# PKU-EPIC/PartManip

Measured on AMD Instinct MI355X. Metric: PPO env-steps/sec (whole node), 4096 envs x 1024-pt clouds, higher is better.
Workload: dtype f32

## Files before the change

### partmanip_amd/csrc/pointnet_enc_screen.h

```cpp
#pragma once

typedef _Float16 ps_f16x8 __attribute__((ext_vector_type(8)));

#define PS_LDP (PN_C2 + 8)
#define PS_CAP 256
#define PS_NW 8
#define PS_P3 (16 * 16 * 64 * 8)
#define PS_OFF_P3 0
#define PS_OFF_W3 (2 * PS_P3)
#define PS_OFF_EPS (PS_OFF_W3 + PN_C3 * PN_C2 * 4)
#define PS_OFF_INV (PS_OFF_EPS + PN_C3 * 4)
#define PS_PACKED_BYTES (PS_OFF_INV + PN_C3 * 4)
#ifndef PS_ABLATE
#define PS_ABLATE 0
#endif
#ifndef PS_SCHED_DEFAULT
#define PS_SCHED_DEFAULT 0
#endif

extern "C" size_t pm_pointnet_packed_screen_bytes(void) { return PS_PACKED_BYTES; }

__device__ __forceinline__ unsigned ps_cvt_pk(float a, float b) {
    unsigned r;
    asm("v_cvt_pk_f16_f32 %0, %1, %2" : "=v"(r) : "v"(a), "v"(b));
    return r;
}

__global__ __launch_bounds__(PN_C2) void ps_pack_kernel(const float* __restrict__ W3, const float* __restrict__ b3,
                                                         unsigned char* __restrict__ packed) {
    __shared__ double Ls[PN_C2], Rs[PN_C2], Ss[PN_C2];
    __shared__ float Ms[PN_C2];
    const int c = blockIdx.x, k = threadIdx.x;
    const float w = W3[c * PN_C2 + k];
    const float aw = fabsf(w);
    Ls[k] = (double)aw;
    Ms[k] = aw < INFINITY ? aw : 0.f;
    __syncthreads();
    for (int o = PN_C2 / 2; o > 0; o >>= 1) {
        if (k < o) {
            Ls[k] += Ls[k + o];
            Ms[k] = fmaxf(Ms[k], Ms[k + o]);
        }
        __syncthreads();
    }
    int ex = -200;
    if (Ms[0] > 0.f) frexpf(Ms[0], &ex);
    const int s = min(15 - ex, 126);
    const float ws = ldexpf(w, s);
    const _Float16 w16 = (_Float16)ws;
    const float wf = (float)w16, d = fabsf(ws - wf);
    Rs[k] = (double)(fabsf(wf) < 0x1p-14f ? fmaxf(fabsf(ws), d) : d);
    Ss[k] = (double)fabsf(wf);
    __syncthreads();
    for (int o = PN_C2 / 2; o > 0; o >>= 1) {
        if (k < o) {
            Rs[k] += Rs[k + o];
            Ss[k] += Ss[k + o];
        }
        __syncthreads();
    }
    const int nb = c >> 5, li = c & 31, step = k >> 4, lq = (k >> 3) & 1, e = k & 7;
    ((_Float16*)(packed + PS_OFF_P3))[(((nb * 16 + step) * 64) + lq * 32 + li) * 8 + e] = w16;
    ((float*)(packed + PS_OFF_W3))[c * PN_C2 + k] = w;
    if (k == 0) {
        const double ed = ((Rs[0] + 0x1p-12 * Ss[0]) * ldexp(1.0, -s) + 1024.0 * 0x1p-24 * (Ls[0] + fabs((double)b3[c]))) * (1.0 + 0x1p-10) + 0x1p-116;
        float ef = (float)ed;
        if ((double)ef < ed) ef = __uint_as_float(__float_as_uint(ef) + 1);
        ((float*)(packed + PS_OFF_EPS))[c] = ef;
        ((float*)(packed + PS_OFF_INV))[c] = ldexpf(1.f, -s);
    }
}

extern "C" int pm_pointnet_pack_weights_screen(const float* W3, const float* b3, void* packed, void* stream) {
    PM_REQUIRE(W3 && b3 && packed);
    if (((uintptr_t)packed & 15) != 0) return PM_EALIGN;
    hipLaunchKernelGGL(ps_pack_kernel, dim3(PN_C3), dim3(PN_C2), 0, pm_stream(stream), W3, b3, (unsigned char*)packed);
    PM_CHECK_LAUNCH();
    return PM_OK;
}

#define PS_MFMA(a, b, c) __builtin_amdgcn_mfma_f32_32x32x16_f16((a), (b), (c), 0, 0, 0)
__device__ __forceinline__ ps_f16x8 ps_h(const uint4& v) { return *(const ps_f16x8*)&v; }

__device__ __forceinline__ void ps_stream(const unsigned short* __restrict__ A, const uint4* __restrict__ B, f32x16 (&acc)[2][2]) {
    uint4 b0[2], b1[2], b2[2], b3[2], a0[2], a1[2];
#pragma unroll
    for (int nb = 0; nb < 2; ++nb) {
        b0[nb] = B[(size_t)(nb * 16 + 0) * 64];
        b1[nb] = B[(size_t)(nb * 16 + 1) * 64];
        b2[nb] = B[(size_t)(nb * 16 + 2) * 64];
    }
#pragma unroll
    for (int mb = 0; mb < 2; ++mb) a0[mb] = *(const uint4*)(A + mb * 32 * PS_LDP);
#define PS_STEP(S_, AC, AN, BC, BN, PFA, PFB)                                                  \
    {                                                                                          \
        if (PFA) {                                                                             \
            _Pragma("unroll") for (int mb = 0; mb < 2; ++mb)                                   \
                AN[mb] = *(const uint4*)(A + mb * 32 * PS_LDP + ((S_) + 1) * 16);              \
        }                                                                                      \
        if (PFB) {                                                                             \
            _Pragma("unroll") for (int nb = 0; nb < 2; ++nb)                                   \
                BN[nb] = B[(size_t)(nb * 16 + (S_) + 3) * 64];                                 \
        }                                                                                      \
        __builtin_amdgcn_sched_barrier(0);                                                     \
        _Pragma("unroll") for (int nb = 0; nb < 2; ++nb)                                       \
            _Pragma("unroll") for (int mb = 0; mb < 2; ++mb)                                   \
                acc[mb][nb] = PS_MFMA(ps_h(AC[mb]), ps_h(BC[nb]), acc[mb][nb]);                \
        __builtin_amdgcn_sched_barrier(0);                                                     \
    }
#pragma unroll 1
    for (int s = 0; s < 12; s += 4) {
        PS_STEP(s, a0, a1, b0, b3, 1, 1)
        PS_STEP(s + 1, a1, a0, b1, b0, 1, 1)
        PS_STEP(s + 2, a0, a1, b2, b1, 1, 1)
        PS_STEP(s + 3, a1, a0, b3, b2, 1, 1)
    }
    PS_STEP(12, a0, a1, b0, b3, 1, 1)
    PS_STEP(13, a1, a0, b1, b0, 1, 0)
    PS_STEP(14, a0, a1, b2, b1, 1, 0)
    PS_STEP(15, a1, a0, b3, b2, 0, 0)
#undef PS_STEP
}

template <int SCHED>
__device__ __forceinline__ bool ps_late_wave(int wave) { return SCHED == 1 && __builtin_amdgcn_readfirstlane(wave) >= 4; }

template <int NT>
__device__ __forceinline__ void ps_copy_h2(const float* __restrict__ H, float* __restrict__ dst, int tid) {
#pragma unroll 2
    for (int i = 0; i < PN_TM * PN_C2 / 4 / NT; ++i) {
        const int q = tid + NT * i, row = q >> 6, c4 = q & 63;
        const f32x4 v = *(const f32x4*)(H + row * PN_LD2 + 4 * c4);
        *(f32x4*)(dst + row * PN_C2 + 4 * c4) = v;
    }
}

static_assert(PN_TM * PN_MAXC == PS_NW * 64, "one staged slot per thread");
__device__ __forceinline__ float ps_point_load(const float* __restrict__ xb, int tile, int C, int tid) {
    const int p = tid >> 3, d = tid & 7;
    return d < C ? xb[(tile * PN_TM + p) * C + d] : 0.f;
}
__device__ __forceinline__ void ps_point_store(float v, int sub_mean, const float (&cen)[3], int tid, float* __restrict__ Xs) {
    const int d = tid & 7;
    if (sub_mean && d < 3) v -= cen[d];
    Xs[tid] = v;
}

#ifdef PS_PROFILE
__device__ unsigned long long ps_prof[4 * 16 * PS_NW * 16];
extern "C" int pm_debug_ps_prof_read(void* dst) {
    return hipMemcpyFromSymbol(dst, HIP_SYMBOL(ps_prof), sizeof(ps_prof)) == hipSuccess ? 0 : 1;
}
#define PS_STAMP(i)                                                                                         \
    if (b < 4 && tile < 16 && lane0 == 0) ps_prof[((b * 16 + tile) * PS_NW + wave) * 16 + (i)] = __builtin_readcyclecounter()
#else
#define PS_STAMP(i)
#endif

template <int CT, int SCHED>
__global__ __launch_bounds__(PS_NW * 64, 2) void pn_fwd_screen_kernel(
    const float* __restrict__ x, long ldx, int P, int C, int sub_mean, const float* __restrict__ W1,
    const float* __restrict__ b1, const float* __restrict__ b2, const float* __restrict__ b3,
    const float* __restrict__ packed, const unsigned char* __restrict__ packed_s, int max_mean, float* __restrict__ feat,
    long ldf, int32_t* __restrict__ argmax, float* __restrict__ h2_save, unsigned long long* __restrict__ counters) {
    constexpr int NT = PS_NW * 64;
    __shared__ __attribute__((aligned(16))) float H[PN_TM * PN_LD2];
    __shared__ __attribute__((aligned(16))) unsigned short Hh[PN_TM * PS_LDP];
    __shared__ __attribute__((aligned(16))) float Xs[PN_TM * PN_MAXC];
    __shared__ double red[16];
    __shared__ double cs[PN_C2];
    __shared__ int skey[PS_NW][PS_CAP];

    const int b = blockIdx.x, tid = threadIdx.x, lane0 = tid & 63, wave = tid >> 6;
    const float* xb = x + (long)b * ldx;
    const float4* P2v = (const float4*)(packed + PN_P2_OFF);
    const float4* P3v = (const float4*)(packed + PN_P3_OFF);
    const uint4* S3 = (const uint4*)(packed_s + PS_OFF_P3);
    const float* W3r = (const float*)(packed_s + PS_OFF_W3);
    const float* epsg = (const float*)(packed_s + PS_OFF_EPS);
    const float* invg = (const float*)(packed_s + PS_OFF_INV);

    float cen[3] = {0.f, 0.f, 0.f};
    if (sub_mean) cloud_centroid<NT>(xb, P, C, red, cen);

    float vmax = -INFINITY, pois = 0.f;
    int imax = 0;
    double csum = 0.0;

    const int li0 = lane0 & 31;
    const float b2r = b2[wave * 32 + li0];
    const float b3r[2] = {b3[(wave * 2 + 0) * 32 + li0], b3[(wave * 2 + 1) * 32 + li0]};
    const float epsr[2] = {epsg[(wave * 2 + 0) * 32 + li0], epsg[(wave * 2 + 1) * 32 + li0]};
    const float invr[2] = {invg[(wave * 2 + 0) * 32 + li0], invg[(wave * 2 + 1) * 32 + li0]};
    float w1r[4] = {0.f, 0.f, 0.f, 0.f}, b1r = 0.f;
    if constexpr (CT == 3 || CT == 4) layer1_row<CT>(W1, b1, w1r, b1r);

    const int ntiles = P / PN_TM;
    stage_points<PN_TM, NT>(xb, 0, C, sub_mean, cen, Xs);
    for (int tile = 0; tile < ntiles; ++tile) {
        int lane = lane0;
        asm volatile("" : "+v"(lane));
        const int li = lane & 31, lh = lane >> 5;
        PS_STAMP(0);
        __syncthreads();
        float xnext = 0.f;
        if (tile + 1 < ntiles) xnext = ps_point_load(xb, tile + 1, C, tid);
        if (!(PS_ABLATE & 1)) {
            if constexpr (CT == 3 || CT == 4) layer1_tile<CT, PN_TM, NT, true>(Xs, w1r, b1r, H);
            else layer1_tile<CT, PN_TM, NT, true>(Xs, W1, b1, C, H);
        }
        PS_STAMP(1);
        __syncthreads();
        {
            f32x16 acc2[2][1];
            zero_acc<2, 1>(acc2);
            if (PS_ABLATE & 2) {
#pragma unroll
                for (int mb = 0; mb < 2; ++mb)
#pragma unroll
                    for (int r = 0; r < 16; ++r)
                        acc2[mb][0][r] = H[(mb * 32 + (r & 3) + 8 * (r >> 2) + 4 * lh) * PN_LD1 + ((wave * 32 + li) & 127)];
            } else {
                layer2_mfma<2, 1>(H, P2v, wave, lane, acc2);
            }
            PS_STAMP(2);
            __syncthreads();
            PS_STAMP(3);
            const int col = wave * 32 + li;
            const float b2c = b2r;
            float ts = 0.f;
            const bool planes = !(PS_ABLATE & 8) || tile == 0;
            const bool odd = (lane & 1) != 0;
            unsigned* Hh2 = (unsigned*)(Hh + (odd ? PS_LDP : 0) + (col & ~1));
#pragma unroll
            for (int mb = 0; mb < 2; ++mb)
#pragma unroll
                for (int r = 0; r < 16; r += 2) {
                    const float z0 = acc2[mb][0][r] + b2c, z1 = acc2[mb][0][r + 1] + b2c;
                    f32x2 v2;
                    if (PS_ABLATE & 4) {
                        v2.x = z0;
                        v2.y = z1;
                    } else {
                        v2 = pm_tanh2(z0, z1);
                    }
                    const int row0 = mb * 32 + (r & 3) + 8 * (r >> 2) + 4 * lh;
                    H[row0 * PN_LD2 + col] = v2.x;
                    H[(row0 + 1) * PN_LD2 + col] = v2.y;
                    ts += v2.x;
                    ts += v2.y;
                    const float own = odd ? v2.y : v2.x, send = odd ? v2.x : v2.y;
                    const float recv = __int_as_float(__builtin_amdgcn_update_dpp(0, __float_as_int(send), 0xB1, 0xf, 0xf, false));
                    const float a = odd ? recv : own, c = odd ? own : recv;
                    if (planes) Hh2[row0 * (PS_LDP / 2)] = ps_cvt_pk(a, c);
                }
            ts += __shfl_xor(ts, 32, 64);
            csum += (double)ts;
            if (tile + 1 < ntiles) ps_point_store(xnext, sub_mean, cen, tid, Xs);
        }
        PS_STAMP(4);
        __syncthreads();
        PS_STAMP(5);

        const bool copy = h2_save && !(PS_ABLATE & 128), late = ps_late_wave<SCHED>(wave);
        float* h2dst = copy ? h2_save + ((long)b * P + (long)tile * PN_TM) * PN_C2 : nullptr;
        if (copy && late) ps_copy_h2<NT>(H, h2dst, tid);

        f32x16 acc[2][2];
        if (PS_ABLATE & 16) {
#pragma unroll
            for (int nb = 0; nb < 2; ++nb)
#pragma unroll
                for (int mb = 0; mb < 2; ++mb)
#pragma unroll
                    for (int r = 0; r < 16; ++r)
                        acc[mb][nb][r] = b3r[nb] + H[(mb * 32 + (r & 3) + 8 * (r >> 2) + 4 * lh) * PN_LD2 + ((wave * 64 + nb * 32 + li) & 255)];
        } else {
            zero_acc<2, 2>(acc);
            ps_stream(Hh + li * PS_LDP + lh * 8, S3 + (size_t)(wave * 2 * 16) * 64 + lane, acc);
        }
        PS_STAMP(6);

        unsigned msk[2];
        float tmax[2];
#if (PS_ABLATE & 32) && defined(__HIP_DEVICE_COMPILE__)
#pragma unroll
        for (int nb = 0; nb < 2; ++nb) {
#pragma unroll
            for (int mb = 0; mb < 2; ++mb) asm volatile("" ::"v"(acc[mb][nb]));
            msk[nb] = 0;
            tmax[nb] = 0.f;
        }
#else
#pragma unroll
        for (int nb = 0; nb < 2; ++nb) {
            float m = -INFINITY;
            const float iv = invr[nb], b3c = b3r[nb];
#pragma unroll
            for (int mb = 0; mb < 2; ++mb)
#pragma unroll
                for (int r = 0; r < 16; ++r) {
                    if (!(PS_ABLATE & 16)) acc[mb][nb][r] = fmaf(acc[mb][nb][r], iv, b3c);
                    m = fmaxf(m, acc[mb][nb][r]);
                }
            m = fmaxf(m, __shfl_xor(m, 32, 64));
            const float e = epsr[nb];
            const float vm = __shfl(vmax, nb * 32 + li, 64);
            const float thr = m - 2.f * e;
            unsigned k = 0;
#pragma unroll
            for (int mb = 0; mb < 2; ++mb)
#pragma unroll
                for (int r = 0; r < 16; ++r) {
                    const float z = acc[mb][nb][r];
                    const bool s = !(z < thr) && !(z + e <= vm);
                    k |= (s ? 1u : 0u) << (mb * 16 + r);
                }
            msk[nb] = k;
            tmax[nb] = m;
        }
#endif
        const int n = __popc(msk[0]) + __popc(msk[1]);
        int incl = n;
#pragma unroll
        for (int o = 1; o < 64; o <<= 1) {
            const int t = __shfl_up(incl, o, 64);
            if (lane >= o) incl += t;
        }
        const int total = __builtin_amdgcn_readlane(incl, 63);
        PS_STAMP(7);

        if (PS_ABLATE & 64) {
            vmax = fmaxf(vmax, lh ? tmax[1] : tmax[0]);
            if (counters && lane == 0) atomicAdd(counters + 0, (unsigned long long)total);
        } else if (total <= PS_CAP) {
            int off = incl - n;
#pragma unroll
            for (int nb = 0; nb < 2; ++nb) {
                unsigned m = msk[nb];
                while (m) {
                    const int bit = __ffs(m) - 1;
                    m &= m - 1;
                    const int row = (bit >> 4) * 32 + (bit & 3) + 8 * ((bit & 15) >> 2) + 4 * lh;
                    skey[wave][off++] = (row << 6) | (nb * 32 + li);
                }
            }
            __builtin_amdgcn_wave_barrier();
            const int j = lane & 7, g = lane >> 3;
            for (int e0 = 0; e0 < total; e0 += 8) {
                const int e = e0 + g;
                const int key = (e < total) ? skey[wave][e] : 0;
                const int row = key >> 6, cl = key & 63;
                const float* hp = H + row * PN_LD2 + 4 * j;
                const float* wp = W3r + (size_t)(wave * 64 + cl) * PN_C2 + 4 * j;
                float s = 0.f;
#pragma unroll
                for (int i = 0; i < 8; ++i) {
                    const float4 w = *(const float4*)(wp + 32 * i);
                    const float4 h = *(const float4*)(hp + 32 * i);
                    s = fmaf(w.x, h.x, s);
                    s = fmaf(w.y, h.y, s);
                    s = fmaf(w.z, h.z, s);
                    s = fmaf(w.w, h.w, s);
                }
                s += __shfl_xor(s, 4, 64);
                s += __shfl_xor(s, 2, 64);
                s += __shfl_xor(s, 1, 64);
                s += b3[wave * 64 + cl];
#pragma unroll
                for (int gg = 0; gg < 8; ++gg)
                    if (e0 + gg < total) {
                        const int kk = __builtin_amdgcn_readlane(key, gg * 8);
                        const float v = __int_as_float(__builtin_amdgcn_readlane(__float_as_int(s), gg * 8));
                        if ((kk & 63) == lane) {
                            const int p = tile * PN_TM + (kk >> 6);
                            if (!(fabsf(v) < INFINITY)) pois += v;
                            if (v > vmax || (v == vmax && p < imax)) {
                                vmax = v;
                                imax = p;
                            }
                        }
                    }
            }
            if (counters) {
                const unsigned long long h0 = __ballot(msk[0] != 0), h1 = __ballot(msk[1] != 0);
                if (lane == 0) {
                    atomicAdd(counters + 0, (unsigned long long)total);
                    atomicAdd(counters + 2, (unsigned long long)(__popc((unsigned)(h0 | (h0 >> 32))) + __popc((unsigned)(h1 | (h1 >> 32)))));
                }
            }
        } else {
#pragma unroll
            for (int nb = 0; nb < 2; ++nb) {
                const float b3c = b3r[nb];
#pragma unroll
                for (int r = 0; r < 16; ++r) acc[0][nb][r] = acc[1][nb][r] = b3c;
            }
            mfma_stream<2, 2, 32>(H + li * PN_LD2 + lh * 128, PN_LD2, P3v + (size_t)(wave * 2) * 32 * 64 + lane, acc);
#pragma unroll
            for (int nb = 0; nb < 2; ++nb) {
                float bv = -INFINITY, ps = 0.f;
                int bp = 0;
#pragma unroll
                for (int mb = 0; mb < 2; ++mb)
#pragma unroll
                    for (int r = 0; r < 16; ++r) {
                        const float v = acc[mb][nb][r];
                        if (!(fabsf(v) < INFINITY)) ps += v;
                        if (v > bv) {
                            bv = v;
                            bp = tile * PN_TM + mb * 32 + (r & 3) + 8 * (r >> 2) + 4 * lh;
                        }
                    }
                const float ov = __shfl_xor(bv, 32, 64), os = __shfl_xor(ps, 32, 64);
                const int op = __shfl_xor(bp, 32, 64);
                if (ov > bv || (ov == bv && op < bp)) {
                    bv = ov;
                    bp = op;
                }
                if (lh == nb) {
                    pois += ps + os;
                    if (bv > vmax || (bv == vmax && bp < imax)) {
                        vmax = bv;
                        imax = bp;
                    }
                }
            }
            if (counters && lane == 0) atomicAdd(counters + 1, 1ull);
        }
        PS_STAMP(8);
        if (copy && !late) ps_copy_h2<NT>(H, h2dst, tid);
        PS_STAMP(9);
    }
    if ((lane0 >> 5) == 0) cs[wave * 32 + lane0] = csum;
    __syncthreads();
    const int ch = tid;
    float v = vmax;
    if (pois != pois) v = pois;
    feat[(long)b * ldf + ch] = v;
    argmax[(long)b * PN_C3 + ch] = imax;
    if (max_mean) {
        const float* wr = W3r + (size_t)ch * PN_C2;
        double s = 0.0;
#pragma unroll 4
        for (int k = 0; k < PN_C2; k += 4) {
            const float4 w = *(const float4*)(wr + k);
            s = fma((double)w.x, cs[k], s);
            s = fma((double)w.y, cs[k + 1], s);
            s = fma((double)w.z, cs[k + 2], s);
            s = fma((double)w.w, cs[k + 3], s);
        }
        float mv = (float)(s / (double)P + (double)b3[ch]);
        if (pois != pois) mv = pois;
        feat[(long)b * ldf + PN_C3 + ch] = mv;
    }
}

extern "C" int pm_pointnet_enc_fwd_screen_sched_f32(const float* x, long ldx, int B, int P, int C, int sub_mean, const float* W1,
                                                    const float* b1, const float* b2, const float* b3, const float* packed,
                                                    const void* packed_screen, int max_mean, float* feat, long ldf,
                                                    int32_t* argmax, float* h2_save, unsigned long long* counters, int schedule,
                                                    void* stream) {
    PM_REQUIRE(x && W1 && b1 && b2 && b3 && packed && packed_screen && feat && argmax);
    PM_REQUIRE(schedule == 0 || schedule == 1);
    if (h2_save && ((uintptr_t)h2_save & 15) != 0) return PM_EALIGN;
    PM_REQUIRE(B > 0 && P > 0 && P % PN_TM == 0 && C >= 1 && C <= PN_MAXC && ldx >= (long)P * C);
    PM_REQUIRE(ldf >= PN_C3 * (max_mean ? 2 : 1));
    PM_REQUIRE(!sub_mean || C >= 3);
    if (((uintptr_t)packed & 15) != 0 || ((uintptr_t)packed_screen & 15) != 0 || ((uintptr_t)counters & 7) != 0) return PM_EALIGN;
#define PS_LAUNCH(CT, S)                                                                                              \
    hipLaunchKernelGGL((pn_fwd_screen_kernel<CT, S>), dim3(B), dim3(PS_NW * 64), 0, pm_stream(stream), x, ldx, P, C, sub_mean, \
                       W1, b1, b2, b3, packed, (const unsigned char*)packed_screen, max_mean, feat, ldf, argmax, h2_save,   \
                       counters)
    if (schedule == 0) {
        if (C == 3) PS_LAUNCH(3, 0);
        else if (C == 4) PS_LAUNCH(4, 0);
        else PS_LAUNCH(0, 0);
    } else {
        if (C == 3) PS_LAUNCH(3, 1);
        else if (C == 4) PS_LAUNCH(4, 1);
        else PS_LAUNCH(0, 1);
    }
#undef PS_LAUNCH
    PM_CHECK_LAUNCH();
    return PM_OK;
}

extern "C" int pm_pointnet_enc_fwd_screen_f32(const float* x, long ldx, int B, int P, int C, int sub_mean, const float* W1,
                                              const float* b1, const float* b2, const float* b3, const float* packed,
                                              const void* packed_screen, int max_mean, float* feat, long ldf,
                                              int32_t* argmax, float* h2_save, unsigned long long* counters, void* stream) {
    return pm_pointnet_enc_fwd_screen_sched_f32(x, ldx, B, P, C, sub_mean, W1, b1, b2, b3, packed, packed_screen, max_mean, feat,
                                                ldf, argmax, h2_save, counters, PS_SCHED_DEFAULT, stream);
}
```

Measured before the change: 36200.

## Track per-channel argmax via packed LDS atomic max and DPP reductions

Replaces the per-lane running max/argmax registers with a shared-memory array of packed 64-bit keys (order-preserving float bits plus inverted point index) updated by workgroup-scope atomic max. This removes the serial readlane/broadcast loop in the exact rescoring path, which now runs only when a non-finite value appears. It also swaps shuffle-based prefix-sum and 8-lane reductions for DPP row operations. The change adds LDS traffic and atomics per candidate and needs careful handling of NaN, -0 and ties.

```diff
diff --git a/partmanip_amd/csrc/pointnet_enc_screen.h b/partmanip_amd/csrc/pointnet_enc_screen.h
--- a/partmanip_amd/csrc/pointnet_enc_screen.h
+++ b/partmanip_amd/csrc/pointnet_enc_screen.h
@@ -146,6 +146,45 @@
     Xs[tid] = v;
 }
 
+#define PS_DPP(old, src, ctrl, rows, banks) __builtin_amdgcn_update_dpp((old), (src), (ctrl), (rows), (banks), false)
+
+__device__ __forceinline__ float ps_sum8(float s) {
+    const int si = __float_as_int(s);
+    int t = PS_DPP(si, si, 0x114, 0xf, 0xa);
+    t = PS_DPP(t, si, 0x104, 0xf, 0x5);
+    s += __int_as_float(t);
+    s += __int_as_float(PS_DPP(0, __float_as_int(s), 0x4e, 0xf, 0xf));
+    s += __int_as_float(PS_DPP(0, __float_as_int(s), 0xb1, 0xf, 0xf));
+    return s;
+}
+
+__device__ __forceinline__ int ps_prefix64(int v) {
+    v += PS_DPP(0, v, 0x111, 0xf, 0xf);
+    v += PS_DPP(0, v, 0x112, 0xf, 0xf);
+    v += PS_DPP(0, v, 0x114, 0xf, 0xf);
+    v += PS_DPP(0, v, 0x118, 0xf, 0xf);
+    v += PS_DPP(0, v, 0x142, 0xa, 0xf);
+    v += PS_DPP(0, v, 0x143, 0xc, 0xf);
+    return v;
+}
+
+#define PS_BEST_INIT 0x007fffffffffffffull
+__device__ __forceinline__ unsigned long long ps_best_pack(float v, int p) {
+    const unsigned u = __float_as_uint(v);
+    const bool nz = u == 0x80000000u;
+    const unsigned hi = nz ? 0x80000000u : u ^ ((unsigned)((int)u >> 31) | 0x80000000u);
+    const unsigned lo = ((0x7fffffffu - (unsigned)p) << 1) | (nz ? 0u : 1u);
+    return ((unsigned long long)hi << 32) | lo;
+}
+__device__ __forceinline__ float ps_best_value(unsigned hi, unsigned lo) {
+    const unsigned u = (hi & 0x80000000u) ? hi ^ 0x80000000u : ~hi;
+    return __uint_as_float((lo & 1u) ? u : 0x80000000u);
+}
+__device__ __forceinline__ int ps_best_point(unsigned lo) { return (int)(0x7fffffffu - (lo >> 1)); }
+__device__ __forceinline__ void ps_best_max(unsigned long long* slot, float v, int p) {
+    __hip_atomic_fetch_max(slot, ps_best_pack(v, p), __ATOMIC_RELAXED, __HIP_MEMORY_SCOPE_WORKGROUP);
+}
+
 #ifdef PS_PROFILE
 __device__ unsigned long long ps_prof[4 * 16 * PS_NW * 16];
 extern "C" int pm_debug_ps_prof_read(void* dst) {
@@ -170,6 +209,7 @@
     __shared__ double red[16];
     __shared__ double cs[PN_C2];
     __shared__ int skey[PS_NW][PS_CAP];
+    __shared__ unsigned long long best[PS_NW][64];
 
     const int b = blockIdx.x, tid = threadIdx.x, lane0 = tid & 63, wave = tid >> 6;
     const float* xb = x + (long)b * ldx;
@@ -183,8 +223,8 @@
     float cen[3] = {0.f, 0.f, 0.f};
     if (sub_mean) cloud_centroid<NT>(xb, P, C, red, cen);
 
-    float vmax = -INFINITY, pois = 0.f;
-    int imax = 0;
+    float pois = 0.f;
+    best[wave][lane0] = PS_BEST_INIT;
     double csum = 0.0;
 
     const int li0 = lane0 & 31;
@@ -283,6 +323,7 @@
 
         unsigned msk[2];
         float tmax[2];
+        const unsigned bhi[2] = {(unsigned)(best[wave][li] >> 32), (unsigned)(best[wave][32 + li] >> 32)};
 #if (PS_ABLATE & 32) && defined(__HIP_DEVICE_COMPILE__)
 #pragma unroll
         for (int nb = 0; nb < 2; ++nb) {
@@ -305,7 +346,7 @@
                 }
             m = fmaxf(m, __shfl_xor(m, 32, 64));
             const float e = epsr[nb];
-            const float vm = __shfl(vmax, nb * 32 + li, 64);
+            const float vm = ps_best_value(bhi[nb], 1u);
             const float thr = m - 2.f * e;
             unsigned k = 0;
 #pragma unroll
@@ -321,17 +362,13 @@
         }
 #endif
         const int n = __popc(msk[0]) + __popc(msk[1]);
-        int incl = n;
-#pragma unroll
-        for (int o = 1; o < 64; o <<= 1) {
-            const int t = __shfl_up(incl, o, 64);
-            if (lane >= o) incl += t;
-        }
+        const int incl = ps_prefix64(n);
         const int total = __builtin_amdgcn_readlane(incl, 63);
         PS_STAMP(7);
 
         if (PS_ABLATE & 64) {
-            vmax = fmaxf(vmax, lh ? tmax[1] : tmax[0]);
+            const float tm = lh ? tmax[1] : tmax[0];
+            if (tm == tm) ps_best_max(&best[wave][lane], tm, 0);
             if (counters && lane == 0) atomicAdd(counters + 0, (unsigned long long)total);
         } else if (total <= PS_CAP) {
             int off = incl - n;
@@ -363,24 +400,20 @@
                     s = fmaf(w.z, h.z, s);
                     s = fmaf(w.w, h.w, s);
                 }
-                s += __shfl_xor(s, 4, 64);
-                s += __shfl_xor(s, 2, 64);
-                s += __shfl_xor(s, 1, 64);
-                s += b3[wave * 64 + cl];
-#pragma unroll
-                for (int gg = 0; gg < 8; ++gg)
-                    if (e0 + gg < total) {
-                        const int kk = __builtin_amdgcn_readlane(key, gg * 8);
-                        const float v = __int_as_float(__builtin_amdgcn_readlane(__float_as_int(s), gg * 8));
-                        if ((kk & 63) == lane) {
-                            const int p = tile * PN_TM + (kk >> 6);
-                            if (!(fabsf(v) < INFINITY)) pois += v;
-                            if (v > vmax || (v == vmax && p < imax)) {
-                                vmax = v;
-                                imax = p;
-                            }
+                s = ps_sum8(s);
+                const float b3s = b3[wave * 64 + cl];
+                s = s == 0.f ? b3s : s + b3s;
+                const bool live = e < total;
+                if (live && j == 0 && s == s) ps_best_max(&best[wave][cl], s, tile * PN_TM + row);
+                if (__any(live && !(fabsf(s) < INFINITY))) {
+#pragma unroll
+                    for (int gg = 0; gg < 8; ++gg)
+                        if (e0 + gg < total) {
+                            const int kk = __builtin_amdgcn_readlane(key, gg * 8);
+                            const float v = __int_as_float(__builtin_amdgcn_readlane(__float_as_int(s), gg * 8));
+                            if ((kk & 63) == lane && !(fabsf(v) < INFINITY)) pois += v;
                         }
-                    }
+                }
             }
             if (counters) {
                 const unsigned long long h0 = __ballot(msk[0] != 0), h1 = __ballot(msk[1] != 0);
@@ -420,10 +453,7 @@
                 }
                 if (lh == nb) {
                     pois += ps + os;
-                    if (bv > vmax || (bv == vmax && bp < imax)) {
-                        vmax = bv;
-                        imax = bp;
-                    }
+                    ps_best_max(&best[wave][lane], bv, bp);
                 }
             }
             if (counters && lane == 0) atomicAdd(counters + 1, 1ull);
@@ -435,7 +465,9 @@
     if ((lane0 >> 5) == 0) cs[wave * 32 + lane0] = csum;
     __syncthreads();
     const int ch = tid;
-    float v = vmax;
+    const unsigned long long bq = best[ch >> 6][ch & 63];
+    float v = ps_best_value((unsigned)(bq >> 32), (unsigned)bq);
+    const int imax = ps_best_point((unsigned)bq);
     if (pois != pois) v = pois;
     feat[(long)b * ldf + ch] = v;
     argmax[(long)b * PN_C3 + ch] = imax;
```

Result: faster. 38670, median of 6 (+6.8%).
